# mcx/AgileRL

Measured on AMD Instinct MI355X. Metric: population env-steps/sec + learner updates/sec, 8-agent PPO at 1/2/4/8 MI355X, higher is better.
Workload: dtype f32 (GAE carry f64); 1 GPU; config 2: one 8-agent PPO population sharded 8 agents per GPU, 128 vec envs per agent, T=16, batch 128, 4 epochs, MLP enc[64]->64 + heads[64] (shared encoder), tournament every 5 iterations; population=8, pop_per_gpu=8, num_envs=128, learn_step=2048, batch_size=128, update_epochs=4, learner=fused, parallelism=population-sharded x1

## Files before the change

agilerl_amd/_lib.py:

```python

from __future__ import annotations

import ctypes
import os

import torch

_HERE = os.path.dirname(os.path.abspath(__file__))
LIB_PATH = os.environ.get("AGX_LIB") or os.path.join(_HERE, "lib", "libagx.so")

_P = ctypes.c_void_p
_I = ctypes.c_int64
_D = ctypes.c_double
_F = ctypes.c_float
_INT = ctypes.c_int
_SZ = ctypes.c_size_t


class AgxMultiHead(ctypes.Structure):
    _fields_ = [("K", ctypes.c_int32), ("nvec", ctypes.c_int32 * 32)]


SIGNATURES = {
    "agx_last_error": (ctypes.c_char_p, []),
# ... 28 lines not shown
    "agx_ppo_act_gauss_graph_workspace_bytes": (_SZ, [_P, _I, _I]),
    "agx_ppo_act_gauss_graph": (_INT, [_P, _I, _I, _I, _P, _P, _I, _INT, ctypes.c_uint64, ctypes.c_uint64, _P, _P, _P,
                                       _P, _I, _P, _P, _P, _P, _P, _P]),
    "agx_ppo_rollout_gauss_graph_max_workgroups": (_I, []),
    "agx_ppo_rollout_gauss_graph_persistent": (_INT, [_P, _I, _I, _I, _P, _P, _I, ctypes.c_uint32, ctypes.c_uint64,
                                                      ctypes.c_uint64, _P, _P, _P, _P, _D, _P, _P]),
    "agx_ppo_eval_gauss_graph_persistent": (_INT, [_P, _I, _I, _I, _P, _P, _P, _P, _P, _P, _I, ctypes.c_uint32,
                                                   ctypes.c_uint64, ctypes.c_uint64, _P, _P, _D, _P, _P]),
    "agx_ppo_gauss_loss_fwd_bwd": (_INT, [_P] * 9 + [_I, _I, _I, _F, _F, _F, _P, _P, _P, _P, _P]),
    "agx_ppo_gauss_graph_check": (_INT, [_P, _I]),
    "agx_ppo_learn_gauss_graph_workspace_bytes": (_SZ, [_P, _I, _I, _I, _I, _I]),
    "agx_ppo_learn_gauss_graph": (_INT, [_P, _I, _P, _P, _P]),
    "agx_ppo_act_multi_graph_workspace_bytes": (_SZ, [_P, _I, _I]),
    "agx_ppo_act_multi_graph": (_INT, [_P, AgxMultiHead, _I, _I, _P, _P, _I, _P, _I, _INT, ctypes.c_uint64,
                                       ctypes.c_uint64, _P, _P, _P, _P, _I, _P, _P, _P, _P]),
    "agx_ppo_rollout_multi_graph_max_workgroups": (_I, []),
    "agx_ppo_rollout_multi_graph_persistent": (_INT, [_P, AgxMultiHead, _I, _I, _P, _P, _I, ctypes.c_uint32,
                                                      ctypes.c_uint64, ctypes.c_uint64, _P, _P, _D, _P, _P]),
    "agx_ppo_eval_multi_graph_persistent": (_INT, [_P, AgxMultiHead, _I, _I, _P, _P, _P, _P, _I, ctypes.c_uint32,
                                                   ctypes.c_uint64, ctypes.c_uint64, _P, _P, _D, _P, _P]),
    "agx_ppo_multi_loss_fwd_bwd": (_INT, [_P, _P, AgxMultiHead] + [_P] * 7 + [_I, _I, _F, _F, _F, _P, _P, _P, _P]),
    "agx_ppo_multi_graph_check": (_INT, [_P, AgxMultiHead]),
    "agx_ppo_learn_multi_graph_workspace_bytes": (_SZ, [_P, AgxMultiHead, _I, _I, _I, _I]),
    "agx_ppo_learn_multi_graph": (_INT, [_P, AgxMultiHead, _P, _P, _P]),
    "agx_ppo_act_bern_graph_workspace_bytes": (_SZ, [_P, _I, _I]),
    "agx_ppo_act_bern_graph": (_INT, [_P, _I, _I, _P, _P, _I, _P, _I, _INT, ctypes.c_uint64, ctypes.c_uint64, _P, _P,
                                      _P, _P, _I, _P, _P, _P, _P]),
    "agx_ppo_rollout_bern_graph_max_workgroups": (_I, []),
    "agx_ppo_rollout_bern_graph_persistent": (_INT, [_P, _I, _I, _P, _P, _I, ctypes.c_uint32, ctypes.c_uint64,
                                                     ctypes.c_uint64, _P, _P, _D, _P, _P]),
    "agx_ppo_eval_bern_graph_persistent": (_INT, [_P, _I, _I, _P, _P, _P, _P, _I, ctypes.c_uint32, ctypes.c_uint64,
                                                  ctypes.c_uint64, _P, _P, _D, _P, _P]),
    "agx_ppo_bern_loss_fwd_bwd": (_INT, [_P, _P, ctypes.c_int32] + [_P] * 7 + [_I, _I, _F, _F, _F, _P, _P, _P, _P]),
    "agx_ppo_bern_graph_check": (_INT, [_P]),
    "agx_ppo_learn_bern_graph_workspace_bytes": (_SZ, [_P, _I, _I, _I, _I]),
    "agx_ppo_learn_bern_graph": (_INT, [_P, _P, _P, _P]),
    "agx_ppo_learn": (_INT, [_P, _P, _P, _P]),
    "agx_ppo_act": (_INT, [_P, _I, _I, _P, _P, _I, _P, _I, _INT, ctypes.c_uint64, ctypes.c_uint64, _P, _P, _P, _P,
                           _I, _P, _P, _P]),
    "agx_ppo_rollout_step": (_INT, [_P, _I, _I, _P, _P, _INT, _INT, ctypes.c_uint64, ctypes.c_uint64, _P]),
    "agx_rollout_workgroups": (_I, [_I, _I]),
    "agx_rollout_max_workgroups": (_I, [_P]),
    "agx_rollout_ctl_bytes": (_SZ, [_I, _I]),
    "agx_rollout_args_bytes": (_SZ, [_I]),
    "agx_ppo_rollout_persistent": (_INT, [_P, _I, _I, _P, _P, _I, ctypes.c_uint32, ctypes.c_uint64, ctypes.c_uint64,
                                          _P, _P, _D, _P]),
    "agx_ppo_eval_persistent": (_INT, [_P, _I, _I, _P, _P, _P, _P, _P, _I, ctypes.c_uint32, ctypes.c_uint64,
                                       ctypes.c_uint64, _P, _P, _D, _P]),
    "agx_host_alloc": (_P, [_SZ]),
    "agx_host_free": (_INT, [_P]),
    "agx_stream_create": (_P, []),
    "agx_host_signal": (_INT, [_P, ctypes.c_uint32]),
    "agx_host_wait": (_INT, [_P, _I, ctypes.c_uint32, _D]),
    "agx_host_signal_range": (_INT, [_P, _I, _I, ctypes.c_uint32]),
    "agx_host_wait_range": (_INT, [_P, _I, _I, ctypes.c_uint32, _D]),
    "agx_host_signal_wait_range": (_INT, [_P, _I, _I, ctypes.c_uint32, _I, _I, ctypes.c_uint32, _D]),
    "agx_per_workspace_bytes": (_SZ, [_I, _I]),
    "agx_per_init": (_INT, [_P, _P, _I, _P]),
    "agx_per_add": (_INT, [_P, _P, _I, _I, _I, _I, _D, _P, _P, _P]),
    "agx_per_update": (_INT, [_P, _P, _I, _I, _P, _P, _I, _D, _D, _P, _P, _P]),
    "agx_per_sample": (_INT, [_P, _P, _I, _P, _I, _I, _D, _P, _P, _P, _P]),
    "agx_per_gather": (_INT, [_P, _P, _I, _P, _P]),
    "agx_segtree_workspace_bytes": (_SZ, [_I]),
    "agx_segtree_init": (_INT, [_P, _I, _INT, _P]),
    "agx_segtree_set": (_INT, [_P, _I, _INT, _P, _P, _I, _P, _P]),
    "agx_segtree_operate": (_INT, [_P, _I, _INT, _I, _I, _P, _P]),
    "agx_segtree_retrieve": (_INT, [_P, _I, _P, _I, _P, _P, _P]),
    "agx_td_workspace_bytes": (_SZ, [_I]),
    "agx_td_target": (_INT, [_P] * 6 + [_I, _I, _D, _INT, _P, _P, _P, _P, _P]),
    "agx_maddpg_critic_target": (_INT, [_P] * 4 + [_I, _D, _P, _P, _P, _P, _P]),
    "agx_td3_smooth_actions": (_INT, [_P] * 4 + [_I, _I, _D, _P, _P]),
    "agx_td3_workspace_bytes": (_SZ, [_I]),
    "agx_td3_critic_target": (_INT, [_P] * 6 + [_I, _D] + [_P] * 6),
    "agx_c51_project_loss": (_INT, [_P] * 7 + [_I, _I, _I, _D, _D, _D, _P, _P, _P]),
    "agx_c51_project_loss_rows": (_INT, [_P] * 5 + [_I, _I, _D, _D, _D, _P, _P, _P]),
    "agx_adam_workspace_bytes": (_SZ, [_I, _I]),
    "agx_clip_adam": (_INT, [_P, _P, _P, _P, _I, _I, _P, _INT, _F, _P, _F, _F, _F, _P, _P, _P, _P]),
    "agx_polyak": (_INT, [_P, _P, _I, _F, _P]),
    "agx_noisy_reset": (_INT, [_P, _INT, _P]),
    "agx_noisy_streams_forward": (_INT, [_P, _INT, _INT, _P, _I, _F, _P]),
    "agx_noisy_streams_forward_each": (_INT, [_P, _INT, _INT, _P, _I, _F, _P]),
    "agx_noisy_streams_workspace_bytes": (_SZ, [_P, _INT, _INT, _I]),
    "agx_noisy_streams_backward": (_INT, [_P, _INT, _INT, _P, _I, _F, _P, _P, _P, _P]),
    "agx_conv2d_forward": (_INT, [_P, _P, _INT, _F, _F, _P, _P, _INT, _P, _P]),
    "agx_conv2d_wgrad_workspace_bytes": (_SZ, [_P]),
    "agx_conv2d_backward": (_INT, [_P, _P, _INT, _F, _F, _P, _P, _P, _P, _P, _P, _INT, _P, _P]),
    "agx_rows_gather_workspace_bytes": (_SZ, [_P, _INT, _I]),
    "agx_rows_gather": (_INT, [_P, _P, _INT, _I, _P, _P, _P]),
    "agx_dueling_head_forward": (_INT, [_P, _P, _P, _I, _I, _I, _INT, _P, _P]),
    "agx_dueling_head_backward": (_INT, [_P, _P, _P, _P, _I, _I, _I, _INT, _P, _P, _P]),
    "agx_dueling_head_forward_rows": (_INT, [_P, _P, _P, _I, _I, _I, _INT, _P, _P]),
    "agx_dueling_head_backward_rows": (_INT, [_P, _P, _P, _P, _I, _I, _I, _P, _P, _P]),
    "agx_conv2d_forward_grouped": (_INT, [_P, _I, _P, _I, _INT, _F, _F, _P, _I, _P, _I, _INT, _P, _I, _P]),
    "agx_conv2d_forward_grouped2": (_INT, [_P, _I, _I, _P, _I, _I, _INT, _F, _F, _P, _I, _I, _P, _I, _I, _INT, _P,
                                           _I, _I, _P]),
    "agx_replay_gather": (_INT, [_P, _P, _P, _INT, _P, _I, _I, _P, _P]),
    "agx_conv2d_wgrad_workspace_bytes_grouped": (_SZ, [_P, _I]),
    "agx_conv2d_backward_grouped": (_INT, [_P, _I, _P, _I, _INT, _F, _F, _P, _I, _P, _P, _I, _P, _P, _P,
                                           _INT, _P, _P]),
    "agx_debug_pow": (_INT, [_P, _P, _P, _I, _P]),
    "agx_debug_learn_stamps": (_INT, [_P]),
    "agx_debug_rollout_stamps": (_INT, [_P]),
    "agx_debug_learn_stall": (_INT, [_INT]),
    "agx_host_shuffle_perms": (_INT, [_P, _P, _I, _I, _I, _P, _P]),
    "agx_debug_stream": (_INT, [_P, _P, _I, _INT, _I, _P]),
}
# ... 50 lines not shown
```

agilerl_amd/csrc/learner.hip:

```cpp
#include <cmath>
#include <cstdlib>
#include <type_traits>

#include "agx_common.h"
#include "ppo_gather.h"
#include "rollout.h"

namespace agx {

#ifndef AGX_LEARN_UNIFORM
#define AGX_LEARN_UNIFORM 1
#endif
#ifndef AGX_LEARN_RS2
#define AGX_LEARN_RS2 0
#endif
#ifndef AGX_LEARN_B2_TAGGED
#define AGX_LEARN_B2_TAGGED 1
#endif
#ifndef AGX_LEARN_B2_SWEEP1
#define AGX_LEARN_B2_SWEEP1 1
#endif
#ifndef AGX_LEARN_VEC_EARLY
#define AGX_LEARN_VEC_EARLY 1
#endif
// ... 333 lines not shown
        if (i + 1 < NB) {
#pragma unroll
            for (int j = 0; j < KB / 4; ++j) {
                av[(i + 1) & 1][j] = a(r, (i + 1) * KB + 4 * j + q);
                bv[(i + 1) & 1][j] = b((i + 1) * KB + 4 * j + q, r);
            }
        }
        __builtin_amdgcn_sched_barrier(0);
#pragma unroll
        for (int j = 0; j < KB / 4; ++j)
            acc = __builtin_amdgcn_mfma_f32_16x16x4f32(av[i & 1][j], bv[i & 1][j], acc, 0, 0, 0);
        __builtin_amdgcn_sched_barrier(0);
    }
    return acc;
}

template <class C>
__device__ __forceinline__ int flat_to_lds(int f) {
    constexpr LearnPlan pl = C::plan;
    int l = 0;
#pragma unroll
    for (int b = 0; b < pl.nblk; ++b) {
        constexpr int dummy = 0;
        (void)dummy;
        const Blk k = pl.blk[b];
        if (f >= k.f0 && f < k.f0 + k.len) {
            const int i = f - k.f0;
            l = k.l0 + (i / k.rowlen) * k.ldst + i % k.rowlen;
        }
    }
    return l;
}
template <class C>
__device__ __forceinline__ int lds_to_flat(int l, int &group) {
    constexpr LearnPlan pl = C::plan;
    int f = -1;
    group = 0;
#pragma unroll
    for (int b = 0; b < pl.nblk; ++b) {
        const Blk k = pl.blk[b];
        const int rows = k.len / k.rowlen;
        if (l >= k.l0 && l < k.l0 + rows * k.ldst) {
            const int i = l - k.l0;
            const int c = i % k.ldst;
            if (c < k.rowlen) {
                f = k.f0 + (i / k.ldst) * k.rowlen + c;
                group = f >= pl.f_cw ? 1 : 0;
            }
        }
    }
    return f;
}

template <class C, int SB = kSB>
struct Fwd {
    static constexpr LearnPlan pl = C::plan;
    static_assert(SB == 8 || SB == 16 || SB == 32, "sub-batch rows");
    float *sm;

    template <int F, int split, int xb, int ldx, int rb, int gb, int bb, bool OUT = false>
    __device__ __forceinline__ void ln_rows() {
        constexpr int W = (!OUT && split >= F) ? ((SB == 8 && F % 64 == 0) ? 64 : (SB <= 16 && F % 32 == 0) ? 32 : 16)
                                               : 16;
        constexpr int NC = F / W;
        constexpr int F0 = split < F ? split : F, F1 = F - F0;
        const int lane = vlane(), wave = swave();
        const int sub = lane & (W - 1);
        const int r = wrow<W>(lane, wave);
        if (SB < kSB && r >= SB) return;
        float z[NC];
        float s0 = 0.f, s1 = 0.f;
#pragma unroll
        for (int i = 0; i < NC; ++i) {
            z[i] = sm[pl.l_s2 + r * pl.ld_s + sub + W * i];
            if (W * i < split) s0 += z[i];
            else s1 += z[i];
        }
        const float m0 = wrow_sum<W>(s0) * (1.f / (float)F0);
        const float m1 = F1 > 0 ? wrow_sum<W>(s1) * (1.f / (float)(F1 > 0 ? F1 : 1)) : 0.f;
        float v0 = 0.f, v1 = 0.f;
#pragma unroll
        for (int i = 0; i < NC; ++i) {
            if (W * i < split) v0 += (z[i] - m0) * (z[i] - m0);
            else v1 += (z[i] - m1) * (z[i] - m1);
        }
        const float r0 = 1.f / sqrtf(wrow_sum<W>(v0) / (float)F0 + 1e-5f);
        const float r1 = F1 > 0 ? 1.f / sqrtf(wrow_sum<W>(v1) / (float)(F1 > 0 ? F1 : 1) + 1e-5f) : 0.f;
        if (sub == 0) {
            sm[rb + 2 * r] = r0;
            sm[rb + 2 * r + 1] = r1;
        }
        constexpr int NA = OUT ? pl.A : 1;
        float pa[NA], pv = 0.f;
#pragma unroll
        for (int a = 0; a < NA; ++a) pa[a] = 0.f;
#pragma unroll
        for (int i = 0; i < NC; ++i) {
            const int j = sub + W * i;
            const float xh = W * i < split ? (z[i] - m0) * r0 : (z[i] - m1) * r1;
            sm[xb + r * ldx + j] = xh;
            const float y = gb >= 0 ? relu(xh * sm[gb + j] + sm[bb + j]) : relu(xh);
            sm[pl.l_s1 + r * pl.ld_s + j] = y;
            if constexpr (OUT) {
                if (W * i < split) {
#pragma unroll
                    for (int a = 0; a < NA; ++a) pa[a] += y * sm[pl.l_aow + a * pl.l_aold + j];
                } else {
                    pv += y * sm[pl.l_cow + j - split];
                }
            }
        }
        if constexpr (OUT) {
            float mine = 0.f;
#pragma unroll
            for (int a = 0; a < NA; ++a) {
                const float t = row_sum(pa[a]);
                mine = sub == a ? t : mine;
            }
            pv = row_sum(pv);
            if (sub < NA) sm[pl.l_lg + r * kMaxA + sub] = mine + sm[pl.l_aob + sub];
            if (sub == 0) sm[pl.l_val + r] = pv + sm[pl.l_cob];
        }
    }

    template <int xb, int ldx, int K, int wb, int ldw, int bias, int fout>
    __device__ __forceinline__ void gemm_fwd() {
        constexpr int MT = m_tiles<SB>();
        constexpr int nt = MT * (fout / 16);
        AGX_IDS;
        for (int t = wave; t < nt; t += kNW) {
            const int m0 = (t % MT) * 16, n0 = (t / MT) * 16;
            f4 c = f4{0.f, 0.f, 0.f, 0.f};
            c = mfma_tile<K>(c, [&](int m, int k) { return sm[xb + (m0 + m) * ldx + k]; },
                             [&](int k, int n) { return sm[wb + (n0 + n) * ldw + k]; });
            const float bv = sm[bias + n0 + lr16];
            if (SB >= 16 || lq * 4 < SB) {
#pragma unroll
                for (int i = 0; i < 4; ++i) sm[pl.l_s2 + (m0 + lq * 4 + i) * pl.ld_s + n0 + lr16] = c[i] + bv;
            }
        }
    }

    template <int L, class F>
    __device__ __forceinline__ void enc_layer(F st) {
        constexpr int K = rup(pl.ein[L], 16);
        gemm_fwd<L == 0 ? pl.l_x0 : pl.l_s1, L == 0 ? pl.ld_x0 : pl.ld_s, K, pl.l_ew[L], pl.l_eld[L], pl.l_eb[L],
                 pl.eout[L]>();
        __syncthreads();
        st(8 + 2 * L);
        ln_rows<pl.eout[L], pl.eout[L], pl.l_xe[L], pl.ld_xe[L], pl.l_re[L], pl.eaff[L] ? pl.l_eg[L] : -1,
                pl.l_ebe[L]>();
        __syncthreads();
        st(9 + 2 * L);
// ... 1148 lines not shown
                    int cq[KM];
#pragma unroll
                    for (int q = 0; q < KM; ++q) {
                        const int qc0 = (int)((long long)n4s * q / g.K), qc1 = (int)((long long)n4s * (q + 1) / g.K);
                        const int c = qc0 + tid + r0;
                        cq[q] = (q < g.K && q != kk && c < qc1 && c < n4) ? c : -1;
                        x[q] = cq[q] >= 0 ? __builtin_bit_cast(f4, __builtin_amdgcn_raw_buffer_load_b128(
                                                                        rs, (q * pl.slab + 4 * c) * 4, 0, 16))
                                          : f4{0.f, 0.f, 0.f, 0.f};
                    }
#pragma unroll
                    for (int q = 0; q < KM; ++q)
                        if (cq[q] >= 0) sm4[cq[q]] = x[q];
                }
#endif
                AGX_STAMP(64 + 2);
            }
            __syncthreads();
            AGX_STAMP(64 + 10);
        }
        ++epochs_done;
        {
            const unsigned long long tb = __builtin_bit_cast(unsigned long long, tkl_v);
            const unsigned thi = __builtin_amdgcn_readfirstlane((unsigned)(tb >> 32));
            const unsigned tlo = __builtin_amdgcn_readfirstlane((unsigned)tb);
            const double tkl = __builtin_bit_cast(double, ((unsigned long long)thi << 32) | tlo);
            if (tkl > 0.0 && kl_total / (double)n_done > tkl) break;
        }
    }

#pragma unroll
    for (int i = 0; i < 4 * kUsed4; ++i) {
        const int l = 4 * own_c(i >> 2) + (i & 3);
        if ((vbits >> i) & 1u) {
            int grp;
            const int f = lds_to_flat<C>(l, grp);
            gp[f] = sm[l];
            gm[f] = am[i];
            gv[f] = av[i];
        }
    }
    if constexpr (ST)
        if (g.stamps && b == 0 && tid < 80) g.stamps[tid] = reinterpret_cast<const long long *>(sm + pl.l_stamp)[tid];
    if (tid == 0 && kk == 0) {
        if (loss_out_v) loss_out_v[p] = loss_total / ((float)S * (float)Ep);
        if (kl_out_v) kl_out_v[p] = n_done ? (float)(kl_total / (double)n_done) : 0.f;
        if (epochs_out_v) epochs_out_v[p] = epochs_done;
        *step_v = step0 + n_done;
    }
#undef IC
#undef BC
}

template <class C>
__device__ __forceinline__ void act_body(const ActArgs &g, float *sm, bool resident, long long *st = nullptr) {
    constexpr LearnPlan pl = C::plan;
    const int p = blockIdx.y, n0 = blockIdx.x * kSB;
    const int tid = threadIdx.x, lane = tid & 63, wave = tid >> 6;
    const int nrow = g.N - n0 < kSB ? g.N - n0 : kSB;
    const float *ob = g.obs + (size_t)p * g.obs_pstride + (size_t)n0 * pl.D;
    constexpr int kObsIt = (kSB * pl.D + kNT - 1) / kNT;
    float obv[kObsIt];
#pragma unroll
    for (int k = 0; k < kObsIt; ++k) {
        const int i = tid + k * kNT;
        obv[k] = i < nrow * pl.D ? ld_sys(ob + i) : 0.f;
    }
    const bool prev = g.st_rew && tid < nrow;
    const size_t idx = (size_t)p * g.N + n0 + tid;
    const PrevStep ps = load_prev_step(g, idx, prev);
    if (st && tid == 0) {
        __builtin_amdgcn_s_waitcnt(0);
        st[0] = (long long)__builtin_amdgcn_s_memrealtime() + (long long)(obv[0] != obv[0]);
    }
    if (prev) store_prev_step(g, p, n0 + tid, idx, ps);
    if (g.obs_copy) {
        float *oc = g.obs_copy + (size_t)p * g.obs_copy_pstride + (size_t)n0 * pl.D;
#pragma unroll
        for (int k = 0; k < kObsIt; ++k)
            if (tid + k * kNT < nrow * pl.D) oc[tid + k * kNT] = obv[k];
    }
    if (!g.act) return;
    for (int i = resident ? pl.param_end + tid : tid; i < pl.act_floats; i += kNT) sm[i] = 0.f;
    __syncthreads();
    if (!resident) load_params<C>(sm, g.params + (size_t)p * pl.n, tid);
#pragma unroll
    for (int k = 0; k < kObsIt; ++k) {
        const int i = tid + k * kNT;
        if (i < kSB * pl.D) sm[pl.l_x0 + (i / pl.D) * pl.ld_x0 + i % pl.D] = obv[k];
    }
    __syncthreads();
    Fwd<C> fw{sm};
    fw.run();
    if (st && tid == 0) st[1] = (long long)__builtin_amdgcn_s_memrealtime();
    const int r = wave + kNW * (lane >> 4), a = lane & 15;
    const bool live = r < nrow;
    float lg = a < pl.A ? sm[pl.l_lg + r * kMaxA + a] : -3.0e38f;
    if (g.mask && a < pl.A && live) {
        const size_t mo = (size_t)p * g.mask_pstride + (size_t)(n0 + r) * pl.A + a;
        const unsigned char ok = ld_sys_u8(g.mask + mo);
        if (g.mask_copy) g.mask_copy[(size_t)p * g.mask_copy_pstride + (size_t)(n0 + r) * pl.A + a] = ok;
        if (!ok) lg = -1.0e8f;
    }
    const float mx = row_max(lg);
    const float lse = mx + logf(row_sum(a < pl.A ? expf(lg - mx) : 0.f));
    const float pa = a < pl.A ? expf(lg - lse) : 0.f;
    const float H = -row_sum(a < pl.A ? pa * logf(pa + 1e-8f) : 0.f);
    float score = lg;
    if (g.sample) {
        const unsigned long long env = stream_env(-1, g.env_base, p, g.N, n0 + r);
        score = a < pl.A ? gumbel_score(lg, a, env, g.seed, g.counter) : -3.0e38f;
    }
    const float best = row_max(score);
    const unsigned long long ball = __ballot(score == best);
    const int choice = __builtin_ctz((unsigned)((ball >> (lane & ~15)) & 0xffffu));
    const float lgc = __builtin_bit_cast(
        float, __builtin_amdgcn_ds_bpermute(((lane & ~15) + choice) * 4, __builtin_bit_cast(int, lg)));
    if (live && a == 0) {
        const size_t o = (size_t)p * g.out_pstride + n0 + r;
        if (g.act_out) g.act_out[o] = choice;
        if (g.logp_out) g.logp_out[o] = lgc - lse;
        if (g.ent_out) g.ent_out[o] = H;
        if (g.value_out) g.value_out[o] = sm[pl.l_val + r];
        if (g.act_flat)
            __hip_atomic_store(g.act_flat + (size_t)p * g.N + n0 + r, (long long)choice, __ATOMIC_RELAXED,
                               __HIP_MEMORY_SCOPE_SYSTEM);
    }
    if (st && tid == 0) st[2] = (long long)__builtin_amdgcn_s_memrealtime();
}

template <class C>
__global__ __launch_bounds__(kNT, 1) void ppo_act_kernel(ActArgs g) {
    extern __shared__ __attribute__((aligned(16))) float sm[];
    act_body<C>(g, sm, false);
}

template <class C>
__global__ __launch_bounds__(kNT, 1) void ppo_rollout_persistent_kernel(const ActArgs *steps, int nsteps,
                                                                        agx_rollout_ctl *ctl,
                                                                        unsigned long long timeout_ticks,
                                                                        unsigned base, long long *stamps) {
    extern __shared__ __attribute__((aligned(16))) float sm[];
    constexpr LearnPlan pl = C::plan;
    __shared__ ActArgs s_args;
    __shared__ int s_go;
    const int tid = threadIdx.x;
    const int blk = blockIdx.y * gridDim.x + blockIdx.x;
    unsigned *rel = rollout_release_word(ctl, gridDim.x * gridDim.y, blk);
    constexpr int kArgWords = (int)(sizeof(ActArgs) / 4);
    if (tid == 0)
        __hip_atomic_fetch_add(&ctl->started, 1u, __ATOMIC_RELAXED, __HIP_MEMORY_SCOPE_SYSTEM);
    for (int t = 0; t < nsteps; ++t) {
        long long *st = stamps && blk == 0 && t < 32 ? stamps + 8 * t : nullptr;
        if (st && tid == 0) st[0] = (long long)__builtin_amdgcn_s_memrealtime();
        if (tid < kArgWords)
            reinterpret_cast<unsigned *>(&s_args)[tid] = reinterpret_cast<const unsigned *>(steps + t)[tid];
        if (tid == 0) {
            s_go = wait_release(rel, ctl, base, t, timeout_ticks);
            if (st) st[1] = (long long)__builtin_amdgcn_s_memrealtime();
            if (stamps && t == 5 && blk < 64) stamps[256 + blk] = (long long)__builtin_amdgcn_s_memrealtime();
        }
        __syncthreads();
        if (!s_go) return;
        const ActArgs g = s_args;
        act_body<C>(g, sm, t > 0 && pl.param_end > 0, st ? st + 2 : nullptr);
        step_stores_acked();
        if (st && tid == 0) st[5] = (long long)__builtin_amdgcn_s_memrealtime();
        if (stamps && tid == 0 && t == 5 && blk < 64) stamps[320 + blk] = (long long)__builtin_amdgcn_s_memrealtime();
        publish_done(ctl, blk, base, t);
    }
}

static bool same_layout(const agx_ppo_net *net, const LearnPlan &pl) {
    if (!pl.ok || net->n_params != pl.n || net->critic_start != pl.f_cw) return false;
    for (int e = 0; e < pl.ne; ++e) {
        if (net->enc_w[e] != pl.f_ew[e] || net->enc_b[e] != pl.f_eb[e]) return false;
        if (pl.eaff[e] && (net->enc_ln_w[e] != pl.f_eg[e] || net->enc_ln_b[e] != pl.f_ebe[e])) return false;
    }
    return net->actor_w == pl.f_aw && net->actor_b == pl.f_ab && net->actor_ln_w == pl.f_ag &&
           net->actor_ln_b == pl.f_abe && net->actor_out_w == pl.f_aow && net->actor_out_b == pl.f_aob &&
           net->critic_w == pl.f_cw && net->critic_b == pl.f_cb && net->critic_ln_w == pl.f_cg &&
           net->critic_ln_b == pl.f_cbe && net->critic_out_w == pl.f_cow && net->critic_out_b == pl.f_cob;
}

static bool dims_match(const agx_ppo_net *net, const NetDims &d) {
    if (net->obs_dim != d.D || net->n_actions != d.A || net->n_enc != d.ne) return false;
    if (net->enc_dim[0] != d.D) return false;
    for (int e = 0; e < d.ne; ++e)
        if (net->enc_dim[e + 1] != d.eo[e]) return false;
    return net->head_actor == d.ha && net->head_critic == d.hc;
}

struct Launcher {
    const LearnPlan *plan;
    void (*learn)(const LearnArgs &, int nblocks, size_t lds, hipStream_t, int sb);
    void (*act)(const ActArgs &, dim3 grid, size_t lds, hipStream_t);
    void (*persist)(const ActArgs *, int, agx_rollout_ctl *, unsigned long long, unsigned, long long *, dim3 grid,
                    size_t lds, hipStream_t);
    int (*persist_occupancy)(size_t lds);
};

template <class C>
static void launch_learn(const LearnArgs &a, int nblocks, size_t lds, hipStream_t s, int sb) {
    static bool attr = false;
    if (!attr) {
        (void)hipFuncSetAttribute((const void *)ppo_learn_kernel<C, 8, 1>, hipFuncAttributeMaxDynamicSharedMemorySize,
                                  160 * 1024);
        (void)hipFuncSetAttribute((const void *)ppo_learn_kernel<C, 8>, hipFuncAttributeMaxDynamicSharedMemorySize,
                                  160 * 1024);
        (void)hipFuncSetAttribute((const void *)ppo_learn_kernel<C, 16, 1>, hipFuncAttributeMaxDynamicSharedMemorySize,
                                  160 * 1024);
        (void)hipFuncSetAttribute((const void *)ppo_learn_kernel<C, 16>, hipFuncAttributeMaxDynamicSharedMemorySize,
                                  160 * 1024);
        (void)hipFuncSetAttribute((const void *)ppo_learn_kernel<C, 32>, hipFuncAttributeMaxDynamicSharedMemorySize,
                                  160 * 1024);
        attr = true;
    }
    constexpr int n4s = C::plan.param_end / 4 + 1;
// ... 369 lines not shown
```

agilerl_amd/csrc/rollout.h:

```cpp
#pragma once

#include "agx_common.h"

namespace agx {

__device__ __forceinline__ unsigned mulhilo(unsigned a, unsigned b, unsigned &hi) {
    const unsigned long long prod = (unsigned long long)a * b;
    hi = (unsigned)(prod >> 32);
    return (unsigned)prod;
}
__device__ __forceinline__ uint4 philox(uint4 c, uint2 k) {
#pragma unroll
    for (int i = 0; i < 10; ++i) {
        unsigned h0, h1;
        const unsigned l0 = mulhilo(0xD2511F53u, c.x, h0);
        const unsigned l1 = mulhilo(0xCD9E8D57u, c.z, h1);
        c = make_uint4(h1 ^ c.y ^ k.x, l1, h0 ^ c.w ^ k.y, l0);
        k.x += 0x9E3779B9u;
        k.y += 0xBB67AE85u;
    }
    return c;
}

struct ActArgs {
// ... 46 lines not shown
        if (v == AGX_ROLLOUT_STOP) return false;
        if (v >= base + (unsigned)(t + 1)) return true;
        if (__builtin_amdgcn_s_memrealtime() - t0 > timeout_ticks) {
            __hip_atomic_store(&ctl->timeout, 1u, __ATOMIC_RELAXED, __HIP_MEMORY_SCOPE_SYSTEM);
            return false;
        }
        __builtin_amdgcn_s_sleep(2);
    }
}

__device__ __forceinline__ void step_stores_acked() {
    __builtin_amdgcn_s_waitcnt(0);
    __syncthreads();
}
__device__ __forceinline__ void publish_done(agx_rollout_ctl *ctl, int blk, unsigned base, int t) {
    if (threadIdx.x == 0)
        __hip_atomic_store(rollout_done_words(ctl) + blk, base + (unsigned)(t + 1), __ATOMIC_RELAXED,
                           __HIP_MEMORY_SCOPE_SYSTEM);
}

struct PrevStep {
    float rw;
    unsigned char dn;
};
__device__ __forceinline__ PrevStep load_prev_step(const ActArgs &g, size_t idx, bool on) {
    PrevStep s{0.f, 0};
    if (on) {
        s.rw = ld_sys(g.st_rew + idx);
        s.dn = ld_sys_u8(g.st_done + idx);
    }
    return s;
}
__device__ __forceinline__ void store_prev_step(const ActArgs &g, int p, int env, size_t idx, PrevStep s) {
    g.rew_prev[(size_t)p * g.prev_pstride + env] = s.rw;
    g.done_prev[(size_t)p * g.prev_pstride + env] = s.dn;
    if (g.scores) {
        float sc = g.scores[idx] + s.rw;
        if (s.dn) {
            g.ret_sum[idx] += (double)sc;
            g.episodes[idx] += 1;
            sc = 0.f;
        }
        g.scores[idx] = sc;
    }
}

__device__ __forceinline__ unsigned long long stream_env(long long env_off, const long long *env_base, int p, int N,
                                                         int row) {
    return (env_off >= 0 ? (unsigned long long)env_off
            : env_base   ? (unsigned long long)env_base[p]
                         : (unsigned long long)p * N) +
           row;
}
__device__ __forceinline__ float gumbel_score(float lg, int a, unsigned long long env, unsigned long long seed,
                                              unsigned long long counter) {
    const uint4 rnd = philox(make_uint4((unsigned)env, (unsigned)(env >> 32), (unsigned)counter,
                                        (unsigned)(counter >> 32) ^ ((unsigned)(a >> 2) << 24)),
                             make_uint2((unsigned)seed, (unsigned)(seed >> 32)));
    const unsigned w = (a & 3) == 0 ? rnd.x : (a & 3) == 1 ? rnd.y : (a & 3) == 2 ? rnd.z : rnd.w;
    const float u = ((float)(w >> 8) + 0.5f) * (1.0f / 16777216.0f);
    return lg - logf(-logf(u));
}

inline ActArgs act_step_args(int64_t P, int64_t N, const float *params, const float *obs, int64_t obs_agent_stride,
                             const uint8_t *action_mask, int64_t mask_agent_stride, int sample, uint64_t seed,
                             uint64_t counter, int64_t *actions, float *log_probs, float *values, float *entropy,
                             int64_t out_agent_stride, int64_t *actions_flat, const int64_t *agent_env_base) {
    ActArgs a{};
    a.params = params;
    a.obs = obs;
    a.obs_pstride = obs_agent_stride;
    a.N = (int)N;
    a.P = (int)P;
    a.sample = sample;
    a.seed = seed;
    a.counter = counter;
    a.act_out = reinterpret_cast<long long *>(actions);
    a.logp_out = log_probs;
    a.value_out = values;
    a.ent_out = entropy;
    a.out_pstride = out_agent_stride;
    a.act_flat = reinterpret_cast<long long *>(actions_flat);
    a.act = 1;
    a.mask = action_mask;
    a.mask_pstride = mask_agent_stride;
    a.env_base = reinterpret_cast<const long long *>(agent_env_base);
    return a;
}

inline ActArgs eval_step_args(int D, int A, int64_t P, int64_t N, const float *params, const float *stage_obs,
                              const uint8_t *stage_mask, int64_t *actions_flat, const int64_t *agent_env_base,
                              uint64_t seed, uint64_t counter) {
    return act_step_args(P, N, params, stage_obs, N * (int64_t)D, stage_mask, N * (int64_t)A, 1, seed, counter,
                         nullptr, nullptr, nullptr, nullptr, 0, actions_flat, agent_env_base);
}

inline int check_persistent(bool pointers_ok, int64_t P, int64_t N, int64_t nsteps, uint32_t base, double timeout_s,
                            const char *who) {
    AGX_REQUIRE(pointers_ok && P > 0 && N > 0 && P <= 65535 && nsteps >= 1, "%s: bad arguments", who);
    AGX_REQUIRE((uint64_t)base + (uint64_t)nsteps < AGX_ROLLOUT_STOP, "%s: base wraps", who);
    AGX_REQUIRE(timeout_s > 0 && timeout_s < 3600, "%s: timeout_s out of range", who);
    return AGX_OK;
}

inline unsigned long long seconds_to_ticks(double s) {
    return (unsigned long long)(s * 1e8);
}

inline void fill_rollout_args(ActArgs &a, int D, int A, int64_t P, int64_t N, const float *params,
                              const agx_rollout_io *io, int act, int sample, uint64_t seed, uint64_t counter) {
    a.params = params;
    a.obs = io->stage_obs;
    a.obs_pstride = N * (int64_t)D;
    a.N = (int)N;
// ... 41 lines not shown
```

agilerl_amd/csrc/runtime.hip:

```cpp
#include <chrono>
#include <cstring>

#include "agx_common.h"

namespace agx {
static thread_local char g_err[512] = "";

void set_error(const char *fmt, ...) {
    va_list ap;
    va_start(ap, fmt);
    vsnprintf(g_err, sizeof(g_err), fmt, ap);
    va_end(ap);
}
}

extern "C" const char *agx_last_error(void) { return agx::g_err; }

extern "C" int agx_version(void) { return 100;  }

extern "C" int agx_device_info(int *out3) {
    if (!out3) {
        agx::set_error("agx_device_info: null output");
        return AGX_EINVAL;
    }
// ... 101 lines not shown
        agx::set_error("agx_stream_create: hipStreamCreateWithFlags failed");
        return nullptr;
    }
    return s;
}

extern "C" int agx_host_signal(agx_rollout_ctl *ctl, uint32_t seq) {
    AGX_REQUIRE(ctl, "agx_host_signal: null ctl");
    const unsigned nwg = __atomic_load_n(&ctl->nwg, __ATOMIC_RELAXED);
    for (unsigned w = 0; w < nwg; ++w) __atomic_store_n(agx::rollout_release_word(ctl, nwg, w), seq, __ATOMIC_RELEASE);
    __atomic_store_n(&ctl->seq, seq, __ATOMIC_RELEASE);
    return AGX_OK;
}

extern "C" int agx_host_signal_range(agx_rollout_ctl *ctl, int64_t w0, int64_t w1, uint32_t seq) {
    AGX_REQUIRE(ctl, "agx_host_signal_range: null ctl");
    const unsigned nwg = __atomic_load_n(&ctl->nwg, __ATOMIC_RELAXED);
    AGX_REQUIRE(w0 >= 0 && w0 <= w1 && w1 <= (int64_t)nwg, "agx_host_signal_range: [%lld, %lld) outside %u",
                (long long)w0, (long long)w1, nwg);
    for (int64_t w = w0; w < w1; ++w)
        __atomic_store_n(agx::rollout_release_word(ctl, nwg, (unsigned)w), seq, __ATOMIC_RELEASE);
    return AGX_OK;
}

extern "C" int agx_host_wait_range(const agx_rollout_ctl *ctl, int64_t w0, int64_t w1, uint32_t target,
                                   double timeout_s) {
    AGX_REQUIRE(ctl && w0 >= 0 && w0 < w1, "agx_host_wait_range: bad arguments");
    const uint32_t *done = agx::rollout_done_words(const_cast<agx_rollout_ctl *>(ctl));
    const auto t0 = std::chrono::steady_clock::now();
    int64_t i = w0;
    for (unsigned spin = 0;; ++spin) {
        while (i < w1 && __atomic_load_n(done + i, __ATOMIC_ACQUIRE) >= target) ++i;
        if (i == w1) return AGX_OK;
        if (__atomic_load_n(&ctl->timeout, __ATOMIC_RELAXED)) {
            agx::set_error("agx_host_wait_range: a workgroup timed out waiting for the host");
            return AGX_EHIP;
        }
        if ((spin & 1023) == 1023 &&
            std::chrono::duration<double>(std::chrono::steady_clock::now() - t0).count() > timeout_s) {
            agx::set_error("agx_host_wait_range: %lld of [%lld, %lld) not done after %.1f s", (long long)(w1 - i),
                           (long long)w0, (long long)w1, timeout_s);
            return AGX_EHIP;
        }
        __builtin_ia32_pause();
    }
}

extern "C" int agx_host_signal_wait_range(agx_rollout_ctl *ctl, int64_t s0, int64_t s1, uint32_t seq, int64_t w0,
                                          int64_t w1, uint32_t target, double timeout_s) {
    const int rc = agx_host_signal_range(ctl, s0, s1, seq);
    return rc != AGX_OK ? rc : agx_host_wait_range(ctl, w0, w1, target, timeout_s);
}

extern "C" int agx_host_wait(const agx_rollout_ctl *ctl, int64_t nwg, uint32_t target, double timeout_s) {
    AGX_REQUIRE(ctl && nwg > 0, "agx_host_wait: bad arguments");
    const uint32_t *done = agx::rollout_done_words(const_cast<agx_rollout_ctl *>(ctl));
    const auto t0 = std::chrono::steady_clock::now();
    int64_t i = 0;
    for (unsigned spin = 0;; ++spin) {
        while (i < nwg && __atomic_load_n(done + i, __ATOMIC_ACQUIRE) >= target) ++i;
        if (i == nwg) return AGX_OK;
        if (__atomic_load_n(&ctl->timeout, __ATOMIC_RELAXED)) {
            agx::set_error("agx_host_wait: a rollout workgroup timed out waiting for the host");
            return AGX_EHIP;
        }
        if ((spin & 1023) == 1023 &&
            std::chrono::duration<double>(std::chrono::steady_clock::now() - t0).count() > timeout_s) {
            agx::set_error("agx_host_wait: %lld of %lld workgroups not done after %.1f s", (long long)(nwg - i),
                           (long long)nwg, timeout_s);
            return AGX_EHIP;
        }
        __builtin_ia32_pause();
    }
}
```

agilerl_amd/population/runner.py:

```python

from __future__ import annotations

import ctypes
import os
import weakref

import numpy as np
import torch

from .. import _lib
from .ppo_pop import PPOPopulation


class AgxRolloutIO(ctypes.Structure):

    _fields_ = [
        ("stage_obs", ctypes.c_void_p), ("stage_rew", ctypes.c_void_p), ("stage_done", ctypes.c_void_p),
        ("obs_slot", ctypes.c_void_p), ("obs_agent_stride", ctypes.c_int64),
        ("rewards_prev", ctypes.c_void_p), ("dones_prev", ctypes.c_void_p), ("prev_agent_stride", ctypes.c_int64),
        ("actions", ctypes.c_void_p), ("log_probs", ctypes.c_void_p), ("values", ctypes.c_void_p),
        ("slot_agent_stride", ctypes.c_int64), ("actions_flat", ctypes.c_void_p),
        ("scores", ctypes.c_void_p), ("return_sum", ctypes.c_void_p), ("episodes", ctypes.c_void_p),
        ("stage_mask", ctypes.c_void_p), ("mask_slot", ctypes.c_void_p), ("mask_agent_stride", ctypes.c_int64),
        ("agent_env_base", ctypes.c_void_p),
# ... 261 lines not shown
        self._finish_persistent()

    def _launch_persistent(self, desc):
        pop = self.pop
        P, N, T = pop.P, pop.N, pop.T
        lib = _lib.load()
        ctl = self.ctl_h.data_ptr()
        base = self.seq_base
        if base + T + 1 >= 0xFFFFFFF0:
            torch.cuda.current_stream().synchronize()
            self.ctl_h.zero_()
            base = 0
        if self.head_persistent:
            self._launch_head(lib, base, ctl)
        elif self.graph_persistent:
            from .learner import graph_act_workspace

            gdesc = pop.learn_descriptor()
            ws = graph_act_workspace(pop, gdesc)[1]
            _lib.check(lib.agx_ppo_rollout_graph_persistent(ctypes.byref(gdesc), P, N, pop.params.data.data_ptr(),
                                                            self._ios, T + 1, base, pop.act_seed, pop.act_counter,
                                                            self.args_h.data_ptr(), ctl, self.timeout_s,
                                                            ws.data_ptr(), _lib.stream()),
                       "agx_ppo_rollout_graph_persistent")
        else:
            _lib.check(lib.agx_ppo_rollout_persistent(ctypes.byref(desc), P, N, pop.params.data.data_ptr(),
                                                      self._ios, T + 1, base, pop.act_seed, pop.act_counter,
                                                      self.args_h.data_ptr(), ctl, self.timeout_s, _lib.stream()),
                       "agx_ppo_rollout_persistent")
        self.seq_base = base + T + 1
        self._mark_stats()
        return lib, ctl, base

    def _launch_head(self, lib, base: int, ctl: int) -> None:
        from .learner import act_workspace

        pop = self.pop
        ws = act_workspace(pop, pop.head_descriptor(), pop.head.stem)[1]
        head_persistent(pop, "rollout",
                        (pop.P, pop.N, pop.params.data.data_ptr(), self._ios, pop.T + 1, base, pop.act_seed,
                         pop.act_counter),
                        (self.args_h.data_ptr(), ctl, self.timeout_s, ws.data_ptr(), _lib.stream()),
                        clip=pop.action_clip())

    def _mark_stats(self) -> None:
        if self.stats_event is None:
            self.stats_event = torch.cuda.Event()
        self.stats_event.record()

    def _pace_persistent(self, lib, ctl, base) -> None:
        T = self.pop.T
        try:
            for t in range(T):
                lib.agx_host_signal(ctl, base + t + 1)
                _lib.check(lib.agx_host_wait(ctl, self.n_wg, base + t + 1, self.timeout_s), "agx_host_wait")
                self._env_step()
            lib.agx_host_signal(ctl, base + T + 1)
        except BaseException:
            lib.agx_host_signal(ctl, 0xFFFFFFFF)
            torch.cuda.current_stream().synchronize()
            self.ctl_h.zero_()
            self.seq_base = 0
            raise
        self.pop.act_counter += T
        self.env_steps += self.pop.P * self.pop.N * T

    def _finish_persistent(self) -> None:
        self.last_value_valid = True
        v = self.__dict__.get("_done_views")
        if v is None:
            v = self._done_views = (self.last_done.view(-1), self.term_h.view(torch.uint8))
        v[0].copy_(v[1], non_blocking=True)

    @torch.no_grad()
    def _collect_torch(self) -> None:
        pop, env = self.pop, self.env
        P, N, T = pop.P, pop.N, pop.T
        if not self.started:
            env.reset(out_obs=self.obs_h.numpy())
            self.last_obs.copy_(self.obs_h.view(P, N, -1), non_blocking=True)
            self.started = True
        self.last_value_valid = False
        pop.obs[:, 0].copy_(self.last_obs)
        for t in range(T):
            pop.act_into(t, self.act_d)
            self.act_h.copy_(self.act_d, non_blocking=True)
            self.ev.record()
            self.ev.synchronize()
            self._env_step()
            pop.rewards[:, t].copy_(self.rew_h.view(P, N), non_blocking=True)
            pop.dones[:, t].copy_(self.done_h.view(torch.uint8).view(P, N), non_blocking=True)
            nxt = pop.obs[:, t + 1] if t + 1 < T else self.last_obs
            nxt.copy_(self.obs_h.view(P, N, -1), non_blocking=True)
            r = pop.rewards[:, t].reshape(-1)
            d = pop.dones[:, t].reshape(-1).bool()
            self.scores += r
            self.ret_sum_env += torch.where(d, self.scores, 0.0).double()
            self.episodes_env += d.long()
            self.scores.masked_fill_(d, 0.0)
        gdesc = pop.learn_descriptor()
        if pop.head is not None:
            from .learner import policy_step_head

            policy_step_head(pop, self.last_obs, N * pop.spec.obs_dim, sample=False, counter=0,
                             values=self.last_value, out_agent_stride=N)
            self.last_value_valid = True
        elif gdesc is not None:
            from .learner import policy_step_graph
# ... 2 lines not shown
                              values=self.last_value, out_agent_stride=N)
            self.last_value_valid = True
        self._mark_stats()
        self.last_done.view(-1).copy_(self.term_h.view(torch.uint8), non_blocking=True)
        self.env_steps += P * N * T

    @torch.no_grad()
    def evaluate(self, loop: int = 1, max_steps: int | None = None) -> np.ndarray:
        pop = self.pop
        pop.eval_rounds = getattr(pop, "eval_rounds", 0) + 1
        out = np.zeros((loop, pop.P))
        for k in range(loop):
            d = _EvalDriver(self, k, max_steps)
            if d.can_pipeline():
                d.run_pipelined()
            else:
                run_lockstep([d])
            out[k] = d.result()
        self.after_evaluation()
        return out.mean(0)

    def _eval_staging(self):
        if getattr(self, "_eval_bufs", None) is None:
            pop = self.pop
            P, N, D = pop.P, pop.N, pop.spec.obs_dim
            lib = _lib.load()
            _, obs, rew, done = _packed(P, N, D, owner=self)
            act = self._coherent_actions()
            ctl = _coherent(self, max(self._ctl_bytes(), int(lib.agx_ppo_rollout_graph_ctl_bytes(P, N))))
            args = _coherent(self, int(lib.agx_rollout_args_bytes(_EVAL_CHUNK)))
            agents = _coherent(self, int(lib.agx_ppo_eval_multi_bytes(P)))
            self._eval_bufs = (obs, rew, done, act, ctl, args, agents)
        return self._eval_bufs

    def after_evaluation(self) -> None:
        self.started = False
        self.last_value_valid = False
        self.scores.zero_()

    def iteration(self) -> torch.Tensor:
        desc = self.pop.fused_descriptor()
        if (self.persistent and desc is not None) or self.graph_persistent:
            return self._iteration_pipelined(desc)
        self.collect()
        self.pop.finish_rollout(self.last_obs, self.last_done,
                                self.last_value if self.last_value_valid else None)
        return self.pop.learn()

    @torch.no_grad()
    def _iteration_pipelined(self, desc) -> torch.Tensor:
        c = self.begin_iteration()
        try:
            while c.t < self.pop.T:
                self.pace_release(c)
                self.pace_wait_step(c)
        except BaseException:
            self.abort_iteration(c)
            raise
        return self.end_iteration(c)

    def begin_iteration(self) -> "_IterCtx":
        desc = self.pop.fused_descriptor()
        if self._ios is None:
            self._build_ios()
        if not self.started:
            self.env.reset(out_obs=self.obs_h.numpy())
            self.started = True
        self.pop.prepare_learn()
        if self._ctl_words is None:
            self._ctl_words = self.ctl_h.numpy().view(np.uint32)
        self._ctl_words[3] = 0
        _pacing_begin()
        try:
            lib, ctl, base = self._launch_persistent(desc)
            self._finish_persistent()
            self.pop.finish_rollout(self.last_obs, self.last_done, self.last_value)
            loss = self.pop.learn(prefetch=False, skip_if_set=ctl + 4)
        except BaseException:
            _pacing_end()
            raise
        return _IterCtx(lib, ctl, base, loss)

    def launch_running(self) -> bool:
        return int(self._ctl_words[3]) >= self.n_wg

    def pace_release(self, c: "_IterCtx") -> None:
        c.lib.agx_host_signal(c.ctl, c.base + c.t + 1)

    def pace_wait_step(self, c: "_IterCtx") -> None:
        _lib.check(c.lib.agx_host_wait(c.ctl, self.n_wg, c.base + c.t + 1, self.timeout_s), "agx_host_wait")
        self._env_step()
        c.t += 1
        if c.t == self.pop.T:
            c.lib.agx_host_signal(c.ctl, c.base + self.pop.T + 1)

    def abort_iteration(self, c: "_IterCtx") -> None:
        try:
            c.lib.agx_host_signal(c.ctl, 0xFFFFFFFF)
            torch.cuda.current_stream().synchronize()
            self.ctl_h.zero_()
            self.seq_base = 0
        finally:
            _pacing_end()

    def end_iteration(self, c: "_IterCtx") -> torch.Tensor:
        self.pop.act_counter += self.pop.T
        self.env_steps += self.pop.P * self.pop.N * self.pop.T
        _pacing_end()
        if self.pop.prefetch_perms:
            self.pop.prefetch_permutations()
        return c.loss


class _IterCtx:

    __slots__ = ("lib", "ctl", "base", "loss", "t")

    def __init__(self, lib, ctl, base, loss):
        self.lib, self.ctl, self.base, self.loss, self.t = lib, ctl, base, loss, 0


_EVAL_CHUNK = 1024


def _eval_nets(runners: list) -> tuple | None:
    descs = [r.pop.eval_descriptor() for r in runners]
    if any(d is None for d in descs):
        return None
    ptrs = [ctypes.cast(ctypes.pointer(d), ctypes.c_void_p).value for r, d in zip(runners, descs) for _ in range(r.pop.P)]
    return (ctypes.c_void_p * len(ptrs))(*ptrs), descs


def population_eval_ok(runners: list, paced: bool = True) -> bool:
    if not runners or (paced and not all(r.persistent or r.graph_persistent for r in runners)):
        return False
    pops = [r.pop for r in runners]
    if len({(p.N, p.spec.obs_dim, p.spec.n_actions) for p in pops}) != 1:
        return False
    if any(p.obs.dtype != torch.float32 for p in pops):
        return False
    nets = _eval_nets(runners)
    if nets is None:
        return False
# ... 402 lines not shown
```

include/agx.h:

```cpp
#ifndef AGX_H
#define AGX_H

#include <stddef.h>
#include <stdint.h>

#ifdef __cplusplus
extern "C" {
#endif

#define AGX_OK 0
#define AGX_EINVAL (-1)
#define AGX_EHIP (-2)
#define AGX_EUNSUPPORTED (-3)

const char *agx_last_error(void);
int agx_version(void);
int agx_device_info(int *out3);

size_t agx_gae_workspace_bytes(int64_t P, int64_t T, int64_t N);
int agx_gae(const float *rewards, const uint8_t *dones, const float *values,
            const float *last_value, const uint8_t *last_done, int64_t P, int64_t T,
            int64_t N, double gamma, double gae_lambda, int use_gae, float *advantages,
            float *returns, double *adv_stats, void *workspace, void *stream);

// ... 52 lines not shown
typedef struct agx_rollout_io {
    const float *stage_obs;
    const float *stage_rew;
    const uint8_t *stage_done;
    float *obs_slot;
    int64_t obs_agent_stride;
    float *rewards_prev;
    uint8_t *dones_prev;
    int64_t prev_agent_stride;
    int64_t *actions;
    float *log_probs, *values;
    int64_t slot_agent_stride;
    int64_t *actions_flat;
    float *scores;
    double *return_sum;
    int64_t *episodes;
    const uint8_t *stage_mask;
    uint8_t *mask_slot;
    int64_t mask_agent_stride;
    const int64_t *agent_env_base;
} agx_rollout_io;
int agx_ppo_rollout_step(const agx_ppo_net *net, int64_t P, int64_t N, const float *params,
                         const agx_rollout_io *io, int act, int sample, uint64_t seed,
                         uint64_t counter, void *stream);

#define AGX_ROLLOUT_ABORT 0xffffffffu
typedef struct agx_rollout_ctl {
    uint32_t seq;
    uint32_t timeout;
    uint32_t nwg;
    uint32_t started;
} agx_rollout_ctl;
#define AGX_ROLLOUT_STOP 0xfffffffeu
int64_t agx_rollout_workgroups(int64_t P, int64_t N);
int64_t agx_rollout_max_workgroups(const agx_ppo_net *net);
size_t agx_rollout_ctl_bytes(int64_t P, int64_t N);
size_t agx_rollout_args_bytes(int64_t nsteps);
int agx_ppo_rollout_persistent(const agx_ppo_net *net, int64_t P, int64_t N, const float *params,
                               const agx_rollout_io *ios, int64_t nsteps, uint32_t base, uint64_t seed,
                               uint64_t counter0, void *args_host, agx_rollout_ctl *ctl, double timeout_s,
                               void *stream);
int agx_ppo_eval_persistent(const agx_ppo_net *net, int64_t P, int64_t N, const float *params,
                            const float *stage_obs, const uint8_t *stage_mask, int64_t *actions_flat,
                            const int64_t *agent_env_base, int64_t nsteps, uint32_t base, uint64_t seed,
                            uint64_t counter0, void *args_host, agx_rollout_ctl *ctl, double timeout_s,
                            void *stream);
int agx_host_shuffle_perms(uint32_t *mt_key, int32_t *mt_pos, int64_t P, int64_t epochs, int64_t S,
                           const int64_t *epochs_per_agent, int64_t *perms);
void *agx_host_alloc(size_t bytes);
int agx_host_free(void *ptr);
void *agx_stream_create(void);
int agx_host_signal(agx_rollout_ctl *ctl, uint32_t seq);
int agx_host_wait(const agx_rollout_ctl *ctl, int64_t nwg, uint32_t target, double timeout_s);
int agx_host_signal_range(agx_rollout_ctl *ctl, int64_t w0, int64_t w1, uint32_t seq);
int agx_host_wait_range(const agx_rollout_ctl *ctl, int64_t w0, int64_t w1, uint32_t target, double timeout_s);
int agx_host_signal_wait_range(agx_rollout_ctl *ctl, int64_t s0, int64_t s1, uint32_t seq, int64_t w0, int64_t w1,
                               uint32_t target, double timeout_s);

size_t agx_per_workspace_bytes(int64_t capacity, int64_t max_batch);
int agx_per_init(double *sum_tree, double *min_tree, int64_t capacity, void *stream);
int agx_per_add(double *sum_tree, double *min_tree, int64_t capacity, int64_t max_size,
                int64_t start, int64_t n, double alpha, const double *max_priority,
                void *workspace, void *stream);
int agx_per_update(double *sum_tree, double *min_tree, int64_t capacity, int64_t max_size,
                   const int64_t *indices, const float *priorities, int64_t n, double alpha,
                   double floor, double *max_priority, void *workspace, void *stream);
int agx_per_sample(const double *sum_tree, const double *min_tree, int64_t capacity,
                   const float *uniforms, int64_t B, int64_t size, double beta,
                   int64_t *indices, float *weights, int32_t *err, void *stream);
int agx_per_gather(const double *tree, const int64_t *nodes, int64_t n, double *out, void *stream);

size_t agx_segtree_workspace_bytes(int64_t capacity);
int agx_segtree_init(double *tree, int64_t capacity, int op, void *stream);
int agx_segtree_set(double *tree, int64_t capacity, int op, const int64_t *indices, const double *values,
                    int64_t n, void *workspace, void *stream);
int agx_segtree_operate(const double *tree, int64_t capacity, int op, int64_t start, int64_t end,
                        double *out, void *stream);
int agx_segtree_retrieve(const double *tree, int64_t capacity, const double *upperbounds, int64_t n,
                         int64_t *indices, int32_t *err, void *stream);

size_t agx_td_workspace_bytes(int64_t B);
int agx_td_target(const float *q_next_online, const float *q_next_target, const float *q_cur,
                  const int64_t *actions, const float *rewards, const float *dones, int64_t B,
                  int64_t A, double gamma, int double_q, float *y, float *g_q, float *loss,
                  void *workspace, void *stream);

int agx_maddpg_critic_target(const float *q, const float *q_next, const float *rewards,
                             const float *dones, int64_t B, double gamma, float *y, float *g_q,
                             float *loss, void *workspace, void *stream);

int agx_c51_project_loss(const float *q_next_online, const float *target_dist,
                         const float *logp_cur, const int64_t *actions, const float *rewards,
                         const float *dones, const float *support, int64_t B, int64_t A,
                         int64_t Z, double v_min, double v_max, double gamma, float *loss,
                         float *proj, void *stream);
int agx_c51_project_loss_rows(const float *target_rows, const float *logp_rows, const float *rewards,
                              const float *dones, const float *support, int64_t B, int64_t Z, double v_min,
                              double v_max, double gamma, float *loss, float *proj, void *stream);

size_t agx_adam_workspace_bytes(int64_t P, int64_t n);
int agx_clip_adam(float *params, float *grads, float *exp_avg, float *exp_avg_sq, int64_t P,
                  int64_t n, const int64_t *group_offsets, int G, float max_norm,
                  const float *lr, float beta1, float beta2, float eps, int64_t *steps,
                  const uint8_t *active, void *workspace, void *stream);
int agx_polyak(float *target, const float *online, int64_t n, float tau, void *stream);
typedef struct agx_noisy_layer {
// ... 61 lines not shown
```

Before: 10.10 million env-steps/s.

## Precompute Gumbel noise before release wait and trim persistent rollout act step

In the persistent rollout kernel, the Philox Gumbel noise for each step is now computed before the workgroup waits on the host release flag, so it is off the critical path. The inference forward skips LayerNorm backward-only stores (normalized activations, reciprocal std) and the per-step LDS zeroing when params are resident. Action stores are gathered through LDS and written by one thread per row. On the host side, signal and wait are merged into a single ctypes call to cut per-step Python overhead. The costs are an extra barrier per step and reliance on the skipped LDS regions not being read by the inference path.

```diff
diff --git a/agilerl_amd/_lib.py b/agilerl_amd/_lib.py
--- a/agilerl_amd/_lib.py
+++ b/agilerl_amd/_lib.py
@@ -104,6 +104,7 @@
     "agx_stream_create": (_P, []),
     "agx_host_signal": (_INT, [_P, ctypes.c_uint32]),
     "agx_host_wait": (_INT, [_P, _I, ctypes.c_uint32, _D]),
+    "agx_host_signal_wait": (_INT, [_P, ctypes.c_uint32, _I, ctypes.c_uint32, _D]),
     "agx_host_signal_range": (_INT, [_P, _I, _I, ctypes.c_uint32]),
     "agx_host_wait_range": (_INT, [_P, _I, _I, ctypes.c_uint32, _D]),
     "agx_host_signal_wait_range": (_INT, [_P, _I, _I, ctypes.c_uint32, _I, _I, ctypes.c_uint32, _D]),
diff --git a/agilerl_amd/csrc/learner.hip b/agilerl_amd/csrc/learner.hip
--- a/agilerl_amd/csrc/learner.hip
+++ b/agilerl_amd/csrc/learner.hip
@@ -409,7 +409,7 @@
     return f;
 }
 
-template <class C, int SB = kSB>
+template <class C, int SB = kSB, bool INF = false>
 struct Fwd {
     static constexpr LearnPlan pl = C::plan;
     static_assert(SB == 8 || SB == 16 || SB == 32, "sub-batch rows");
@@ -443,7 +443,7 @@
         }
         const float r0 = 1.f / sqrtf(wrow_sum<W>(v0) / (float)F0 + 1e-5f);
         const float r1 = F1 > 0 ? 1.f / sqrtf(wrow_sum<W>(v1) / (float)(F1 > 0 ? F1 : 1) + 1e-5f) : 0.f;
-        if (sub == 0) {
+        if (!INF && sub == 0) {
             sm[rb + 2 * r] = r0;
             sm[rb + 2 * r + 1] = r1;
         }
@@ -455,7 +455,7 @@
         for (int i = 0; i < NC; ++i) {
             const int j = sub + W * i;
             const float xh = W * i < split ? (z[i] - m0) * r0 : (z[i] - m1) * r1;
-            sm[xb + r * ldx + j] = xh;
+            if (!INF) sm[xb + r * ldx + j] = xh;
             const float y = gb >= 0 ? relu(xh * sm[gb + j] + sm[bb + j]) : relu(xh);
             sm[pl.l_s1 + r * pl.ld_s + j] = y;
             if constexpr (OUT) {
@@ -1710,8 +1710,9 @@
 #undef BC
 }
 
-template <class C>
-__device__ __forceinline__ void act_body(const ActArgs &g, float *sm, bool resident, long long *st = nullptr) {
+template <class C, bool PS = false>
+__device__ __forceinline__ void act_body(const ActArgs &g, float *sm, bool resident, float noise = 0.f,
+                                         long long *st = nullptr) {
     constexpr LearnPlan pl = C::plan;
     const int p = blockIdx.y, n0 = blockIdx.x * kSB;
     const int tid = threadIdx.x, lane = tid & 63, wave = tid >> 6;
@@ -1739,8 +1740,10 @@
             if (tid + k * kNT < nrow * pl.D) oc[tid + k * kNT] = obv[k];
     }
     if (!g.act) return;
-    for (int i = resident ? pl.param_end + tid : tid; i < pl.act_floats; i += kNT) sm[i] = 0.f;
-    __syncthreads();
+    if (!resident || !PS) {
+        for (int i = resident ? pl.param_end + tid : tid; i < pl.act_floats; i += kNT) sm[i] = 0.f;
+        __syncthreads();
+    }
     if (!resident) load_params<C>(sm, g.params + (size_t)p * pl.n, tid);
 #pragma unroll
     for (int k = 0; k < kObsIt; ++k) {
@@ -1748,7 +1751,7 @@
         if (i < kSB * pl.D) sm[pl.l_x0 + (i / pl.D) * pl.ld_x0 + i % pl.D] = obv[k];
     }
     __syncthreads();
-    Fwd<C> fw{sm};
+    Fwd<C, kSB, PS> fw{sm};
     fw.run();
     if (st && tid == 0) st[1] = (long long)__builtin_amdgcn_s_memrealtime();
     const int r = wave + kNW * (lane >> 4), a = lane & 15;
@@ -1766,8 +1769,12 @@
     const float H = -row_sum(a < pl.A ? pa * logf(pa + 1e-8f) : 0.f);
     float score = lg;
     if (g.sample) {
-        const unsigned long long env = stream_env(-1, g.env_base, p, g.N, n0 + r);
-        score = a < pl.A ? gumbel_score(lg, a, env, g.seed, g.counter) : -3.0e38f;
+        if constexpr (PS) {
+            score = a < pl.A ? lg - noise : -3.0e38f;
+        } else {
+            const unsigned long long env = stream_env(-1, g.env_base, p, g.N, n0 + r);
+            score = a < pl.A ? gumbel_score(lg, a, env, g.seed, g.counter) : -3.0e38f;
+        }
     }
     const float best = row_max(score);
     const unsigned long long ball = __ballot(score == best);
@@ -1780,9 +1787,22 @@
         if (g.logp_out) g.logp_out[o] = lgc - lse;
         if (g.ent_out) g.ent_out[o] = H;
         if (g.value_out) g.value_out[o] = sm[pl.l_val + r];
-        if (g.act_flat)
-            __hip_atomic_store(g.act_flat + (size_t)p * g.N + n0 + r, (long long)choice, __ATOMIC_RELAXED,
-                               __HIP_MEMORY_SCOPE_SYSTEM);
+        if (g.act_flat) {
+            if constexpr (PS)
+                sm[pl.l_lg + r * kMaxA] = __builtin_bit_cast(float, choice);
+            else
+                __hip_atomic_store(g.act_flat + (size_t)p * g.N + n0 + r, (long long)choice, __ATOMIC_RELAXED,
+                                   __HIP_MEMORY_SCOPE_SYSTEM);
+        }
+    }
+    if constexpr (PS) {
+        if (g.act_flat) {
+            __syncthreads();
+            if (tid < nrow)
+                __hip_atomic_store(g.act_flat + (size_t)p * g.N + n0 + tid,
+                                   (long long)__builtin_bit_cast(int, sm[pl.l_lg + tid * kMaxA]), __ATOMIC_RELAXED,
+                                   __HIP_MEMORY_SCOPE_SYSTEM);
+        }
     }
     if (st && tid == 0) st[2] = (long long)__builtin_amdgcn_s_memrealtime();
 }
@@ -1813,6 +1833,15 @@
         if (st && tid == 0) st[0] = (long long)__builtin_amdgcn_s_memrealtime();
         if (tid < kArgWords)
             reinterpret_cast<unsigned *>(&s_args)[tid] = reinterpret_cast<const unsigned *>(steps + t)[tid];
+        __syncthreads();
+        const ActArgs g = s_args;
+        float noise = 0.f;
+        {
+            const int lane = tid & 63, a = lane & 15, r = (tid >> 6) + kNW * (lane >> 4);
+            if (g.act && g.sample && a < pl.A)
+                noise = gumbel_noise(a, stream_env(-1, g.env_base, blockIdx.y, g.N, blockIdx.x * kSB + r), g.seed,
+                                     g.counter);
+        }
         if (tid == 0) {
             s_go = wait_release(rel, ctl, base, t, timeout_ticks);
             if (st) st[1] = (long long)__builtin_amdgcn_s_memrealtime();
@@ -1820,8 +1849,7 @@
         }
         __syncthreads();
         if (!s_go) return;
-        const ActArgs g = s_args;
-        act_body<C>(g, sm, t > 0 && pl.param_end > 0, st ? st + 2 : nullptr);
+        act_body<C, true>(g, sm, t > 0 && pl.param_end > 0, noise, st ? st + 2 : nullptr);
         step_stores_acked();
         if (st && tid == 0) st[5] = (long long)__builtin_amdgcn_s_memrealtime();
         if (stamps && tid == 0 && t == 5 && blk < 64) stamps[320 + blk] = (long long)__builtin_amdgcn_s_memrealtime();
diff --git a/agilerl_amd/csrc/rollout.h b/agilerl_amd/csrc/rollout.h
--- a/agilerl_amd/csrc/rollout.h
+++ b/agilerl_amd/csrc/rollout.h
@@ -122,14 +122,18 @@
                          : (unsigned long long)p * N) +
            row;
 }
-__device__ __forceinline__ float gumbel_score(float lg, int a, unsigned long long env, unsigned long long seed,
+__device__ __forceinline__ float gumbel_noise(int a, unsigned long long env, unsigned long long seed,
                                               unsigned long long counter) {
     const uint4 rnd = philox(make_uint4((unsigned)env, (unsigned)(env >> 32), (unsigned)counter,
                                         (unsigned)(counter >> 32) ^ ((unsigned)(a >> 2) << 24)),
                              make_uint2((unsigned)seed, (unsigned)(seed >> 32)));
     const unsigned w = (a & 3) == 0 ? rnd.x : (a & 3) == 1 ? rnd.y : (a & 3) == 2 ? rnd.z : rnd.w;
     const float u = ((float)(w >> 8) + 0.5f) * (1.0f / 16777216.0f);
-    return lg - logf(-logf(u));
+    return logf(-logf(u));
+}
+__device__ __forceinline__ float gumbel_score(float lg, int a, unsigned long long env, unsigned long long seed,
+                                              unsigned long long counter) {
+    return lg - gumbel_noise(a, env, seed, counter);
 }
 
 inline ActArgs act_step_args(int64_t P, int64_t N, const float *params, const float *obs, int64_t obs_agent_stride,
diff --git a/agilerl_amd/csrc/runtime.hip b/agilerl_amd/csrc/runtime.hip
--- a/agilerl_amd/csrc/runtime.hip
+++ b/agilerl_amd/csrc/runtime.hip
@@ -177,6 +177,13 @@
     return rc != AGX_OK ? rc : agx_host_wait_range(ctl, w0, w1, target, timeout_s);
 }
 
+extern "C" int agx_host_signal_wait(agx_rollout_ctl *ctl, uint32_t seq, int64_t nwg, uint32_t target,
+                                    double timeout_s) {
+    AGX_REQUIRE(ctl, "agx_host_signal_wait: null ctl");
+    const int rc = agx_host_signal(ctl, seq);
+    return rc != AGX_OK ? rc : agx_host_wait(ctl, nwg, target, timeout_s);
+}
+
 extern "C" int agx_host_wait(const agx_rollout_ctl *ctl, int64_t nwg, uint32_t target, double timeout_s) {
     AGX_REQUIRE(ctl && nwg > 0, "agx_host_wait: bad arguments");
     const uint32_t *done = agx::rollout_done_words(const_cast<agx_rollout_ctl *>(ctl));
diff --git a/agilerl_amd/population/runner.py b/agilerl_amd/population/runner.py
--- a/agilerl_amd/population/runner.py
+++ b/agilerl_amd/population/runner.py
@@ -337,8 +337,8 @@
         T = self.pop.T
         try:
             for t in range(T):
-                lib.agx_host_signal(ctl, base + t + 1)
-                _lib.check(lib.agx_host_wait(ctl, self.n_wg, base + t + 1, self.timeout_s), "agx_host_wait")
+                _lib.check(lib.agx_host_signal_wait(ctl, base + t + 1, self.n_wg, base + t + 1, self.timeout_s),
+                           "agx_host_wait")
                 self._env_step()
             lib.agx_host_signal(ctl, base + T + 1)
         except BaseException:
@@ -447,8 +447,7 @@
         c = self.begin_iteration()
         try:
             while c.t < self.pop.T:
-                self.pace_release(c)
-                self.pace_wait_step(c)
+                self.pace_step(c)
         except BaseException:
             self.abort_iteration(c)
             raise
@@ -484,6 +483,14 @@
 
     def pace_wait_step(self, c: "_IterCtx") -> None:
         _lib.check(c.lib.agx_host_wait(c.ctl, self.n_wg, c.base + c.t + 1, self.timeout_s), "agx_host_wait")
+        self._step_released(c)
+
+    def pace_step(self, c: "_IterCtx") -> None:
+        seq = c.base + c.t + 1
+        _lib.check(c.lib.agx_host_signal_wait(c.ctl, seq, self.n_wg, seq, self.timeout_s), "agx_host_wait")
+        self._step_released(c)
+
+    def _step_released(self, c: "_IterCtx") -> None:
         self._env_step()
         c.t += 1
         if c.t == self.pop.T:
diff --git a/include/agx.h b/include/agx.h
--- a/include/agx.h
+++ b/include/agx.h
@@ -128,6 +128,7 @@
 void *agx_stream_create(void);
 int agx_host_signal(agx_rollout_ctl *ctl, uint32_t seq);
 int agx_host_wait(const agx_rollout_ctl *ctl, int64_t nwg, uint32_t target, double timeout_s);
+int agx_host_signal_wait(agx_rollout_ctl *ctl, uint32_t seq, int64_t nwg, uint32_t target, double timeout_s);
 int agx_host_signal_range(agx_rollout_ctl *ctl, int64_t w0, int64_t w1, uint32_t seq);
 int agx_host_wait_range(const agx_rollout_ctl *ctl, int64_t w0, int64_t w1, uint32_t target, double timeout_s);
 int agx_host_signal_wait_range(agx_rollout_ctl *ctl, int64_t s0, int64_t s1, uint32_t seq, int64_t w0, int64_t w1,
```

Result: faster. 10.75 million env-steps/s, median of 6 (+6.4%).
